# Ham3798/shielded-pool-pinocchio-solana

Hardware: AMD Instinct MI355X
Metric: Groth16 proofs/sec (higher is better)
Workload: dtype u32x8 (254-bit Montgomery integers); 1 GPU; audit_circuit (RLWE, const-PK; scripts/generate_audit.py:246-465), batch of 2048 independent proofs per GPU per step, every row a distinct witness; circuit=audit, n_constraints=29178, n_wires=35432, domain=32768, batch_per_gpu=2048, n_distinct_witnesses=2048, table_bytes=226725433344, parallelism=independent proofs x1, pk_bytes=9850060

## Files before the change

include/spp.h:

```cpp
#ifndef SPP_H
#define SPP_H
#include <stddef.h>
#include <stdint.h>
#ifdef __cplusplus
extern "C" {
#endif

#define SPP_OK 0
#define SPP_ERR_BAD_INPUT (-1)
#define SPP_ERR_NO_DEVICE (-2)
#define SPP_ERR_IO (-3)
#define SPP_ERR_UNSAT (-4)
#define SPP_ERR_HIP (-5)
#define SPP_ERR_NOT_IMPLEMENTED (-6)
#define SPP_ERR_FORMAT (-7)

#define SPP_CIRCUIT_WITHDRAW 1
#define SPP_CIRCUIT_AUDIT 2
#define SPP_CIRCUIT_WITHDRAW_REFSHAPE 3
#define SPP_CIRCUIT_WITHDRAW_DEPTH20 4

#define SPP_PROOF_LEN 388
#define SPP_WITHDRAW_PW_LEN 172
#define SPP_AUDIT_PW_LEN 76
// ... 172 lines not shown
int  spp_pool_withdraw_batch(spp_pool*, size_t count, const uint8_t* proofs, const uint8_t* pws, const uint8_t* recipients,
                             int32_t* result, uint64_t* amounts);
#define SPP_INSTR_DEPOSIT 0
#define SPP_INSTR_SUBMIT_AUDIT 1
#define SPP_INSTR_WITHDRAW 2
int  spp_pool_settle_log(spp_pool*, size_t count, const uint8_t* kinds,
                         size_t n_deposits, const uint8_t* roots,
                         size_t n_audits, const uint8_t* audit_proofs, const uint8_t* audit_pws,
                         size_t n_withdraws, const uint8_t* withdraw_proofs, const uint8_t* withdraw_pws, const uint8_t* recipients,
                         int32_t* result, uint64_t* amounts);

int spp_merkle_tree_find(spp_merkle_tree* t, size_t count, const uint8_t* leaves, const uint64_t* from, uint64_t* indices, uint32_t* matches);

#define SPP_WALLET_RECORD_LEN 160
#define SPP_WALLET_IN_TREE  1
#define SPP_WALLET_SPENT    2
#define SPP_WALLET_AUDITED  4
#define SPP_WALLET_REPEATED 8
int spp_wallet_sync(spp_merkle_tree* t, spp_pool* pool , size_t count, const uint8_t* deposits ,
                    const uint8_t* recipients , uint64_t* indices, uint32_t* flags,
                    uint8_t* records , uint8_t* notes );

int spp_ntt_fr(spp_ctx* ctx, uint8_t* data, uint32_t logn, int inverse);
int spp_msm_g1(spp_ctx* ctx, const uint8_t* bases, const uint8_t* scalars, size_t n, int window_bits, uint8_t out[64]);
int spp_msm_g2(spp_ctx* ctx, const uint8_t* bases, const uint8_t* scalars, size_t n, int window_bits, uint8_t out[128]);
int spp_msm_flat_unit(spp_ctx* ctx, int group, const uint8_t* bases, size_t n, const uint8_t* scalars, size_t P, int window_bits, uint8_t* out,
                      uint32_t* redo_lanes);

int spp_msm_g1_pippenger(spp_ctx* ctx, const uint8_t* bases, const uint8_t* scalars, size_t n, uint8_t out[64]);
int spp_msm_g2_pippenger(spp_ctx* ctx, const uint8_t* bases, const uint8_t* scalars, size_t n, uint8_t out[128]);
int spp_msm_g1_pippenger_bench(spp_ctx* ctx, size_t n, uint64_t seed, const uint8_t scale_be[32], int iters, uint8_t out[64],
                               float* ms_total, float* ms_bucket_kernel);
int spp_msm_g1_pippenger_bench_dist(spp_ctx* ctx, size_t n, uint64_t seed, uint32_t small_permille, const uint8_t scale_be[32], int iters,
                                    uint8_t out[64], float* ms_total, float* ms_bucket_kernel);
int spp_msm_g1_pippenger_bench_shard(spp_ctx* ctx, size_t n_total, size_t first, size_t count, uint64_t seed, uint32_t small_permille,
                                     const uint8_t scale_be[32], int iters, uint8_t out[64], float* ms_total, float* ms_bucket_kernel);

#ifdef __cplusplus
}
#endif
#endif
```

shielded-pool-pinocchio-solana_amd/csrc/kernels.hpp:

```cpp
#pragma once
#include <hip/hip_runtime.h>
#include <stdint.h>
#include "bn254.hpp"
#include "f29.hpp"
#include "msm_plan.hpp"
#include "msm_ragged.hpp"
#include "rlwe_ntt.hpp"

namespace spp {

struct DevSparse {
  const uint32_t* rowptr;
  const uint32_t* wire;
  const uint32_t* coeff;
  const uint32_t* lit;
};
static constexpr uint32_t COEFF_ONE = 0x80000000u;
static constexpr uint32_t COEFF_MINUS_ONE = 0x40000000u;
static constexpr uint32_t COEFF_MASK = 0x3fffffffu;

struct HashConsts {
  const Fr* pos3_rc;  const Fr* pos3_mds;
  const Fr* pos5_rc;  const Fr* pos5_mds;
  const Fr* p2_rc;    const Fr* p2_mu;
  const uint32_t* pos3_mds29;
  const uint32_t* pos5_mds29;
};
// ... 124 lines not shown
struct PoolSet;
struct PoolState;
void launch_pool_screen_audit(hipStream_t st, const PoolSet& audits, uint64_t salt, const uint8_t* pws, uint32_t count, int32_t* prov, uint32_t* list,
                              uint32_t* n_list);
void launch_pool_screen_withdraw(hipStream_t st, const PoolState* state, const PoolSet& audits, const PoolSet& nullifiers, uint64_t salt,
                                 const uint8_t* pws, const uint8_t* recipients, uint32_t count, int32_t* prov, uint64_t* amounts, uint32_t* list,
                                 uint32_t* n_list);
struct PoolLogView;
void launch_pool_screen_withdraw_log(hipStream_t st, const PoolLogView& view, const PoolSet& audits, const PoolSet& nullifiers, uint64_t salt,
                                     const uint8_t* pws, const uint8_t* recipients, const uint32_t* deposits_before, const uint32_t* audits_before,
                                     uint32_t count, int32_t* prov, uint64_t* amounts, uint32_t* list, uint32_t* n_list);
void launch_pool_scatter(hipStream_t st, const uint32_t* pos, uint32_t count, const int32_t* codes, int32_t* result, const uint64_t* amounts,
                         uint64_t* amounts_out);
void launch_pool_screen_import(hipStream_t st, const PoolSet& set, uint64_t salt, const uint8_t* keys, uint32_t count, int32_t* prov);
void launch_pool_contains(hipStream_t st, const PoolSet& set, uint64_t salt, const uint8_t* keys, uint32_t count, uint8_t* present);
void launch_pool_resolve(hipStream_t st, uint32_t* slots, uint32_t mask, uint64_t salt, const uint8_t* keys, uint32_t stride, uint32_t count,
                         const int32_t* prov, const int32_t* proof_ok, int32_t dup, int32_t* result);
void launch_pool_commit(hipStream_t st, const PoolSet& set, uint64_t salt, const uint8_t* keys, uint32_t stride, uint32_t count, const int32_t* result,
                        uint32_t* set_count);
void launch_spmv_check(hipStream_t st, DevCircuit dc, const Fr* W, Fr* abc, uint32_t n, uint32_t P, uint32_t* status, int16_t* small = nullptr);

void launch_ntt(hipStream_t st, Fr* data, uint32_t logn, uint32_t P, const Fr* tw, bool dif, uint32_t nbatch, size_t batch_stride,
                const Fr* post = nullptr);
void launch_scale_rows(hipStream_t st, Fr* data, const Fr* table, uint32_t n, uint32_t P, uint32_t nbatch, size_t batch_stride);
void launch_qap_pointwise(hipStream_t st, Fr* abc, uint32_t n, uint32_t P, Fr zinv);
void launch_qap_product(hipStream_t st, Fr* abc, uint32_t n, uint32_t P);

template <class F>
struct MsmWalk;
template <>
struct MsmWalk<Fq> {
  static constexpr uint32_t waves_per_simd = 3;
  static constexpr uint32_t rows_waves_per_simd = 2;
  static constexpr int product_form = F29_SCAN;
  static constexpr uint32_t occ(uint32_t Wt) { return Wt == 1 ? waves_per_simd : rows_waves_per_simd; }
};
template <>
struct MsmWalk<Fq2> {
  static constexpr uint32_t waves_per_simd = 2;
  static constexpr uint32_t rows_waves_per_simd = 1;
  static constexpr int product_form = F29_COLUMNS;
  static constexpr uint32_t occ(uint32_t Wt) { return Wt == 1 ? waves_per_simd : rows_waves_per_simd; }
};
template <class F>
void launch_build_table(hipStream_t st, const Affine<F>* bases, uint32_t N, uint32_t c, uint32_t Wt, uint32_t row0, uint32_t nrows,
                        Affine<F>* table, XYZZ<F>* tmp, F* tmp_pre, const MsmBlock* blocks = nullptr, uint32_t E = 0);
// ... 55 lines not shown
```

shielded-pool-pinocchio-solana_amd/csrc/kernels_ntt.hip:

```cpp
#include "kernels.hpp"

namespace spp {

static constexpr uint32_t NTT_TILE_ELEMS = 1024;
static constexpr uint32_t NTT_THREADS = 256;

template <bool DIF>
__global__ void __launch_bounds__(NTT_THREADS) k_ntt_pass(Fr* __restrict__ data, uint32_t logn, uint32_t P, const Fr* __restrict__ tw,
                                                          uint32_t s_lo, uint32_t s_hi, size_t batch_stride, const Fr* __restrict__ post) {
  extern __shared__ __align__(16) unsigned char smem_raw[];
  Fr* sh = reinterpret_cast<Fr*>(smem_raw);
  data += (size_t)blockIdx.y * batch_stride;
  const uint32_t n = 1u << logn;
  const uint32_t lg = s_hi - s_lo;
  const uint32_t G = 1u << lg;
  const uint32_t T = NTT_TILE_ELEMS / G;
  const uint32_t stride = DIF ? (n >> s_hi) : (1u << s_lo);
  const uint64_t Cq = (uint64_t)stride * P;
  const uint64_t ncols = ((uint64_t)n >> lg) * P;
  const uint64_t col0 = (uint64_t)blockIdx.x * T;
  const bool col_major = Cq >= T;

  if (col_major && T <= NTT_THREADS) {
    const uint32_t tc = threadIdx.x & (T - 1), jr = threadIdx.x / T, jstep = NTT_THREADS / T;
// ... 67 lines not shown
        sh[(j + half_l) * T + tc] = e ? d * tw[e] : d;
      } else {
        if (e) v = v * tw[e];
        sh[j * T + tc] = u + v;
        sh[(j + half_l) * T + tc] = u - v;
      }
    }
    __syncthreads();
  }

  for (uint32_t idx = threadIdx.x; idx < G * T; idx += NTT_THREADS) {
    uint32_t j, tc;
    if (col_major) { tc = idx % T; j = idx / T; } else { j = idx % G; tc = idx / G; }
    uint64_t col = col0 + tc;
    if (col < ncols) {
      uint64_t bh = col / Cq, q = col % Cq;
      Fr v = sh[j * T + tc];
      if (post) v = v * post[(uint32_t)(bh * G) * stride + j * stride + (uint32_t)(q / P)];
      data[bh * G * Cq + (uint64_t)j * Cq + q] = v;
    }
  }
}

void launch_ntt(hipStream_t st, Fr* data, uint32_t logn, uint32_t P, const Fr* tw, bool dif, uint32_t nbatch, size_t batch_stride,
                const Fr* post) {
  static bool attr_set = false;
  if (!attr_set) {
    (void)hipFuncSetAttribute((const void*)k_ntt_pass<true>, hipFuncAttributeMaxDynamicSharedMemorySize, (int)(NTT_TILE_ELEMS * sizeof(Fr)));
    (void)hipFuncSetAttribute((const void*)k_ntt_pass<false>, hipFuncAttributeMaxDynamicSharedMemorySize, (int)(NTT_TILE_ELEMS * sizeof(Fr)));
    attr_set = true;
  }
  uint32_t npass = (logn + 7) / 8;
  uint32_t s = 0;
  for (uint32_t ps = 0; ps < npass; ps++) {
    uint32_t lg = (logn - s + (npass - ps) - 1) / (npass - ps);
    uint32_t G = 1u << lg, T = NTT_TILE_ELEMS / G;
    uint64_t ncols = ((uint64_t)1 << (logn - lg)) * P;
    dim3 grid((uint32_t)((ncols + T - 1) / T), nbatch);
    size_t shmem = (size_t)NTT_TILE_ELEMS * sizeof(Fr);
    if (dif)
      hipLaunchKernelGGL(k_ntt_pass<true>, grid, dim3(NTT_THREADS), shmem, st, data, logn, P, tw, s, s + lg, batch_stride,
                         ps + 1 == npass ? post : (const Fr*)nullptr);
    else
      hipLaunchKernelGGL(k_ntt_pass<false>, grid, dim3(NTT_THREADS), shmem, st, data, logn, P, tw, s, s + lg, batch_stride,
                         ps + 1 == npass ? post : (const Fr*)nullptr);
    s += lg;
  }
}

__global__ void __launch_bounds__(256) k_scale_rows(Fr* __restrict__ data, const Fr* __restrict__ table, uint32_t n, uint32_t P,
                                                    size_t batch_stride) {
  data += (size_t)blockIdx.y * batch_stride;
  uint64_t total = (uint64_t)n * P;
  for (uint64_t g = (uint64_t)blockIdx.x * blockDim.x + threadIdx.x; g < total; g += (uint64_t)gridDim.x * blockDim.x) {
    uint32_t i = (uint32_t)(g / P);
    data[g] = data[g] * table[i];
  }
}
void launch_scale_rows(hipStream_t st, Fr* data, const Fr* table, uint32_t n, uint32_t P, uint32_t nbatch, size_t batch_stride) {
  uint64_t total = (uint64_t)n * P;
  uint32_t blocks = (uint32_t)((total + 255) / 256);
  if (blocks > 2048) blocks = 2048;
  hipLaunchKernelGGL(k_scale_rows, dim3(blocks, nbatch), dim3(256), 0, st, data, table, n, P, batch_stride);
}

__global__ void __launch_bounds__(256) k_qap_pointwise(Fr* __restrict__ abc, uint64_t total, Fr zinv) {
  Fr* a = abc;
  const Fr* b = abc + total;
// ... 24 lines not shown
```

shielded-pool-pinocchio-solana_amd/csrc/spp_circuit.hpp:

```cpp
#pragma once
#include "spp_internal.hpp"
#include "msm_classes.hpp"

template <class F>
struct MsmSet {
  uint32_t N = 0;
  Affine<F>* table = nullptr;
  uint32_t* rows = nullptr;
  bool from_h = false;
  uint32_t c = 0;
  uint32_t Wt = 0;
  MsmBlock* blocks = nullptr;
  bool narrow = false;
};
template <class F>
struct MsmBuf {
  XYZZ<F>* partial = nullptr;
  XYZZ<F>* out = nullptr;
  size_t partial_cap = 0;
  MsmPlan plan{};
};
struct Workspace {
  hipStream_t st = nullptr;
  hipStream_t st2 = nullptr;
// ... 50 lines not shown
  MsmTuning msm;
};
static constexpr uint64_t SCALED_BLIND_MAX_SCALARS = 1500000;
inline uint32_t scaled_blind_max_batch(uint32_t n_a, uint32_t n_b1) {
  const uint64_t n = (uint64_t)n_a + n_b1;
  return n ? (uint32_t)std::max<uint64_t>(1, std::min<uint64_t>(1024, SCALED_BLIND_MAX_SCALARS / n)) : 1;
}
struct spp_circuit {
  spp_ctx* ctx = nullptr;
  std::vector<SolveStep> schedule;
  Circuit circ;
  DevCircuit dc{};
  uint32_t c_bits = 10, n = 0, logn = 0;
  uint32_t max_batch_div = SOLVE_SCRATCH_MIN_ROWS;
  DevCoop coop{};
  Switches sw;
  bool generic_solver = false;
  uint32_t row_r = 0, row_s = 0, row_rs = 0, n_rows = 0;
  size_t in_stride = 0, pw_stride = 0;
  uint64_t table_bytes = 0;
  MsmSet<Fq> A, B1, K, Z, CB, CS;
  MsmSet<Fq2> B2;
  Fr *tw_fwd = nullptr, *tw_inv = nullptr, *coset_br = nullptr, *coset_inv_br = nullptr;
  Fr zinv;
  std::vector<void*> owned;
  Workspace ws[SPP_NWS];
  int next_ws = 0, last_ws = 0, prev_ws = 0;
  std::vector<PendingTable<Fq>> pending1;
  std::vector<PendingTable<Fq2>> pending2;
};

template <class T>
static int own_upload(spp_circuit* c, T** dst, const std::vector<T>& src) {
  HIP_TRY(dev_upload(dst, src));
  c->owned.push_back((void*)*dst);
  return 0;
}

#pragma GCC visibility push(hidden)
int coop_plan(spp_circuit* c);
int row_paths_plan(spp_circuit* c);
void destroy_circuit(spp_circuit* c);
void free_workspace(Workspace& w);
#pragma GCC visibility pop
```

shielded-pool-pinocchio-solana_amd/csrc/spp_load.cpp:

```cpp
#include "spp_circuit.hpp"

static std::vector<PendingTable<Fq>>& pending(spp_circuit* c, Fq*) { return c->pending1; }
static std::vector<PendingTable<Fq2>>& pending(spp_circuit* c, Fq2*) { return c->pending2; }

static int upload_sparse(spp_circuit* c, const Circuit& circ, const Sparse& m, DevSparse* out) {
  std::vector<uint32_t> wire(m.terms.size()), coeff(m.terms.size()), lit(m.terms.size(), 0);
  Fr one = Fr::one(), mone = Fr::one().neg();
  std::vector<uint32_t> small(circ.coeffs.size(), 0);
  for (size_t ci = 0; ci < circ.coeffs.size(); ci++) {
    uint32_t v[8], nv[8];
    circ.coeffs[ci].to_canonical(v);
    bool hi0 = true;
    for (int k = 1; k < 8; k++) hi0 = hi0 && v[k] == 0;
    if (hi0 && v[0] != 0 && v[0] < (1u << 28)) { small[ci] = v[0]; continue; }
    circ.coeffs[ci].neg().to_canonical(nv);
    hi0 = true;
    for (int k = 1; k < 8; k++) hi0 = hi0 && nv[k] == 0;
    if (hi0 && nv[0] != 0 && nv[0] < (1u << 28)) small[ci] = nv[0] | 0x80000000u;
  }
  for (size_t i = 0; i < m.terms.size(); i++) {
    wire[i] = m.terms[i].wire;
    uint32_t ci = m.terms[i].coeff;
    uint32_t flag = 0;
    if (circ.coeffs[ci] == one) flag = COEFF_ONE;
// ... 400 lines not shown
  for (uint32_t k = 0; k < n / 2; k++) {
    tf[k] = a;
    ti[k] = b;
    a = a * w;
    b = b * wi;
  }
  Fr g = c->sw.h_mode == 2 ? fr_root_of_unity(logn + 1) : Fr::from_u64(5), gi = g.inv(), ninv = Fr::from_u64(n).inv();
  std::vector<Fr> gp(n), gip(n);
  Fr x = ninv, y = ninv;
  for (uint32_t i = 0; i < n; i++) {
    gp[i] = x;
    gip[i] = y;
    x = x * g;
    y = y * gi;
  }
  for (uint32_t pos = 0; pos < n; pos++) {
    uint32_t i = bitrev(pos, logn);
    cb[pos] = gp[i];
    cib[pos] = gip[i];
  }
  if ((e = own_upload(c, &c->tw_fwd, tf)) || (e = own_upload(c, &c->tw_inv, ti)) || (e = own_upload(c, &c->coset_br, cb)) ||
      (e = own_upload(c, &c->coset_inv_br, cib)))
    return e;
  Fr gn = g.pow_u64(n);
  c->zinv = (gn - Fr::one()).inv();
  return 0;
}

static int load_key_sets(spp_circuit* c, const LoadState& s) {
  const PkFile& pk = s.pk;
  const uint32_t* cw = s.cw;
  const bool* flat = s.flat;
  int e;
  {
    std::vector<uint32_t> w = pk.A_w;
    std::vector<G1Affine> p = pk.A;
    merge_point(w, p, 0u, pk.alpha1);
    w.push_back(c->row_r); p.push_back(pk.delta1);
    if ((e = make_set(c, &c->A, w, p, false, cw[0], flat[0], msm_base_bounds(s.wc, w)))) return e;
  }
  {
    std::vector<uint32_t> w = pk.B1_w;
    std::vector<G1Affine> p = pk.B1;
    merge_point(w, p, 0u, pk.beta1);
    w.push_back(c->row_s); p.push_back(pk.delta1);
    if ((e = make_set(c, &c->B1, w, p, false, cw[1], flat[1], msm_base_bounds(s.wc, w)))) return e;
// ... 426 lines not shown
```

shielded-pool-pinocchio-solana_amd/csrc/spp_micro_api.cpp:

```cpp
#include "spp_internal.hpp"
#include "arith_probe.hpp"

extern "C" int spp_ntt_fr(spp_ctx* ctx, uint8_t* data, uint32_t logn, int inverse) {
  if (!ctx || !data || logn == 0 || logn > 24) return fail(SPP_ERR_BAD_INPUT, "bad argument");
  std::lock_guard<std::mutex> lk(ctx->mu);
  HIP_TRY(hipSetDevice(ctx->device));
  const uint32_t n = 1u << logn;
  Fr w = fr_root_of_unity(logn);
  if (inverse) w = w.inv();
  std::vector<Fr> tw(n / 2 ? n / 2 : 1), host(n);
  Fr a = Fr::one();
  for (uint32_t k = 0; k < n / 2; k++) { tw[k] = a; a = a * w; }
  for (uint32_t i = 0; i < n; i++) host[i] = Fr::from_bytes_be(data + 32 * (size_t)i);
  DevBuf d_tw, d_x;
  HIP_TRY(d_tw.alloc(sizeof(Fr) * tw.size()));
  HIP_TRY(d_x.alloc(sizeof(Fr) * n));
  HIP_TRY(hipMemcpy(d_tw.p, tw.data(), sizeof(Fr) * tw.size(), hipMemcpyHostToDevice));
  HIP_TRY(hipMemcpy(d_x.p, host.data(), sizeof(Fr) * n, hipMemcpyHostToDevice));
  launch_ntt(ctx->stream, d_x.as<Fr>(), logn, 1, d_tw.as<Fr>(), true, 1, 0);
  HIP_TRY(hipStreamSynchronize(ctx->stream));
  HIP_TRY(hipGetLastError());
  HIP_TRY(hipMemcpy(host.data(), d_x.p, sizeof(Fr) * n, hipMemcpyDeviceToHost));
  Fr ninv = inverse ? Fr::from_u64(n).inv() : Fr::one();
  for (uint32_t pos = 0; pos < n; pos++) {
    Fr v = host[pos];
    if (inverse) v = v * ninv;
    v.to_bytes_be(data + 32 * (size_t)bitrev(pos, logn));
  }
  return SPP_OK;
}

extern "C" int spp_debug_arith(spp_ctx* ctx, uint32_t selector, uint32_t arg, size_t n, const uint32_t* in, size_t in_words, uint32_t* out,
                               size_t out_words) {
  if (!ctx || !in || !out) return fail(SPP_ERR_BAD_INPUT, "NULL argument");
  if (n == 0 || n > ((size_t)1 << 20)) return fail(SPP_ERR_BAD_INPUT, "n must be in [1, 2^20]");
  uint32_t iw = 0, ow = 0;
  if (!arith_probe_shape(selector, &iw, &ow)) return fail(SPP_ERR_BAD_INPUT, "unknown selector 0x%x", selector);
  if (!arith_probe_arg_ok(selector, arg)) return fail(SPP_ERR_BAD_INPUT, "selector 0x%x does not know arg %u", selector, arg);
  if (in_words != iw || out_words != ow)
    return fail(SPP_ERR_BAD_INPUT, "selector 0x%x takes %u words and returns %u per case", selector, iw, ow);
  std::lock_guard<std::mutex> lk(ctx->mu);
  HIP_TRY(hipSetDevice(ctx->device));
  hipStream_t st = ctx->stream;
  DevBuf d_in, d_out;
  UP(d_in, in, n * iw * sizeof(uint32_t));
  HIP_TRY(d_out.alloc(n * ow * sizeof(uint32_t)));
  if (!launch_arith_probe(st, selector, arg, d_in.as<uint32_t>(), d_out.as<uint32_t>(), (uint32_t)n))
    return fail(SPP_ERR_BAD_INPUT, "unknown selector 0x%x", selector);
  HIP_TRY(hipGetLastError());
  HIP_TRY(hipStreamSynchronize(st));
  HIP_TRY(hipMemcpy(out, d_out.p, n * ow * sizeof(uint32_t), hipMemcpyDeviceToHost));
// ... 141 lines not shown
```

shielded-pool-pinocchio-solana_amd/csrc/spp_prove.cpp:

```cpp
#include "spp_circuit.hpp"

template <class T>
static int ws_alloc(Workspace& w, T** p, size_t count) {
  HIP_TRY(hipMalloc((void**)p, sizeof(T) * std::max<size_t>(count, 1)));
  w.owned.push_back((void*)*p);
  return 0;
}
template <class F>
static int ws_set(const spp_circuit* c, Workspace& w, const MsmSet<F>* s, MsmBuf<F>* b, size_t P) {
  b->partial_cap = msm_partial_cap(s->N, P, s->c, s->Wt, MsmWalk<F>::occ(s->Wt), c->sw.msm);
  int e;
  if ((e = ws_alloc(w, &b->partial, b->partial_cap))) return e;
  return ws_alloc(w, &b->out, P);
}
static int ensure_workspace(spp_circuit* c, Workspace& w, size_t P) {
  if (P <= w.cap) return 0;
  HIP_TRY(hipStreamSynchronize(w.st));
  free_workspace(w);
  int e;
  if ((e = ws_alloc(w, &w.W, (size_t)c->n_rows * P)) || (e = ws_alloc(w, &w.abc, (size_t)3 * c->n * P)) ||
      (e = ws_alloc(w, &w.scratch, (size_t)c->max_batch_div * P)) || (e = ws_alloc(w, &w.commit_affine, P)) ||
      (e = ws_alloc(w, &w.d_inputs, c->in_stride * P)) || (e = ws_alloc(w, &w.d_rs, 64 * P)) ||
      (e = ws_alloc(w, &w.d_proofs, (size_t)SPP_PROOF_LEN * P)) || (e = ws_alloc(w, &w.d_pws, c->pw_stride * P)) ||
      (e = ws_alloc(w, &w.d_status, P)) || (e = ws_alloc(w, &w.counters, 256 * P)))
// ... 74 lines not shown
          } else launch_solve_coop(st, c->dc, c->coop, w.W, w.scratch, tr, P);
        }
        else launch_solve(st, c->dc, w.W, w.scratch, s.a, s.b, P);
        break;
      case SolveStep::BATCH_DIV: launch_batch_div(st, c->dc, w.W, w.scratch, s.a, s.b, P); break;
      case SolveStep::COUNT8: launch_count8(st, c->dc, w.W, w.counters, s.a, s.b, s.c, P); break;
      case SolveStep::COMMIT:
        run_msm(c, w, c->CB, w.CB, P, true);
        launch_challenge(st, w.CB.out, w.W, circ.challenge_wire, P, w.commit_affine, d_status);
        break;
    }
  }
  hipEventRecord(w.ev[1], st);
  hipEventRecord(w.ev_w, st);
  hipStream_t side = (w.st2 != w.st && w.own_st2p && P > c->sw.coop_max_batch) ? w.own_st2p : w.st2;
  if (c->sw.no_side && P <= c->sw.coop_max_batch) side = st;
  hipStreamWaitEvent(side, w.ev_w, 0);
  run_msm(c, w, c->B2, w.B2, P, false, side, &w.g2_ev);
  hipEventRecord(w.ev_b2, side);
  launch_spmv_check(st, c->dc, w.W, w.abc, n, P, d_status, w.small);
  hipEventRecord(w.ev[2], st);
  const size_t bs = (size_t)n * P;
  const uint32_t nt = c->sw.h_mode == 2 ? 2 : 3;
  launch_ntt(st, w.abc, c->logn, P, c->tw_inv, true, nt, bs, c->coset_br);
  launch_ntt(st, w.abc, c->logn, P, c->tw_fwd, false, nt, bs);
  if (c->sw.h_mode == 2) launch_qap_product(st, w.abc, n, P);
  else launch_qap_pointwise(st, w.abc, n, P, c->zinv);
  if (c->sw.h_mode == 0) launch_ntt(st, w.abc, c->logn, P, c->tw_inv, true, 1, bs, c->coset_inv_br);
  hipEventRecord(w.ev[3], st);
  {
    MsmFoldSets<Fq> fs{};
    const MsmSet<Fq>* sets[7] = {&c->A, &c->B1, &c->K, &c->Z, &c->CS, &c->A, &c->B1};
    MsmBuf<Fq>* bufs[7] = {&w.A, &w.B1, &w.K, &w.Z, &w.CS, &w.sA, &w.rB};
    const Fr* scal[7] = {nullptr, nullptr, nullptr, nullptr, nullptr, w.Ws, w.Wr};
    const int nsets = scaled_blind ? 7 : 5;
    if (scaled_blind) launch_scale_witness(st, w.W, w.Ws, w.Wr, c->n_rows, c->row_r, c->row_s, P);
    for (int i = 0; i < nsets; i++) {
      run_msm(c, w, *sets[i], *bufs[i], P, i < 5, nullptr, nullptr, false, scal[i]);
      fs.partial[i] = bufs[i]->partial;
      fs.out[i] = bufs[i]->out;
      fs.Sg[i] = sets[i]->N ? bufs[i]->plan.Sg : 0;
      fs.R[i] = bufs[i]->plan.R;
      fs.c[i] = sets[i]->c;
    }
    launch_msm_reduce_multi<Fq>(st, fs, nsets, P);
  }
  hipEventRecord(w.ev[4], st);
  hipStreamWaitEvent(st, w.ev_b2, 0);
  hipEventRecord(w.ev[5], st);
  AssembleArgs a;
  a.mA = w.A.out; a.mB1 = w.B1.out; a.mB2 = w.B2.out; a.mK = w.K.out; a.mZ = w.Z.out; a.mPok = w.CS.out;
// ... 416 lines not shown
```

shielded-pool-pinocchio-solana_amd/spp/lib.py:

```python
import ctypes
import os

_HERE = os.path.dirname(os.path.abspath(__file__))
LIB_PATH = os.path.join(os.path.dirname(_HERE), "libspp.so")
_LIB = None

SPP_OK = 0
SPP_ERR_BAD_INPUT = -1
SPP_ERR_UNSAT = -4
SPP_CIRCUIT_WITHDRAW = 1
SPP_CIRCUIT_AUDIT = 2
SPP_CIRCUIT_WITHDRAW_DEPTH20 = 4
SPP_CIRCUIT_WITHDRAW_REFSHAPE = 3
PROOF_LEN = 388
NOTE_LEN = 160
DEPOSIT_LEN = 96
AUDIT_PW_LEN = 76
SPP_RLC_SERIAL_TAIL = 1
SPP_RLC_NO_FALLBACK = 2
SPP_AUDIT_BAD_PROOF = 1
SPP_AUDIT_BAD_CIPHERTEXT = 2
SPP_AUDIT_BAD_IDENTITY = 4
WITHDRAW_PW_LEN = 172
SPP_POOL_STATE_LEN = 1072
# ... 110 lines not shown
    L.spp_pool_set_verifier.argtypes = [vp, i32, u32]
    L.spp_pool_verify_stats.argtypes = [vp, ctypes.POINTER(u32)]
    L.spp_pool_new.argtypes = [vp, cp, sz, cp, sz, ctypes.c_uint64, ctypes.POINTER(vp)]
    L.spp_pool_free.argtypes = [vp]
    L.spp_pool_free.restype = None
    L.spp_pool_add_roots.argtypes = [vp, sz, cp]
    L.spp_pool_state.argtypes = [vp, vp]
    L.spp_pool_counts.argtypes = [vp, vp]
    L.spp_pool_import_keys.argtypes = [vp, i32, sz, cp]
    L.spp_pool_contains.argtypes = [vp, i32, sz, cp, vp]
    L.spp_pool_submit_audit_batch.argtypes = [vp, sz, cp, cp, vp]
    L.spp_pool_withdraw_batch.argtypes = [vp, sz, cp, cp, cp, vp, vp]
    L.spp_pool_settle_log.argtypes = [vp, sz, cp, sz, cp, sz, cp, cp, sz, cp, cp, cp, vp, vp]
    L.spp_withdraw_rows_from_tree.argtypes = [vp, sz, cp, vp]
    L.spp_prove_withdraw_notes_device.argtypes = [vp, vp, sz, vp, vp, vp, vp, vp]
    L.spp_prove_withdraw_notes.argtypes = [vp, vp, sz, cp, cp, vp, vp, vp]
    L.spp_shamir_reconstruct.argtypes = [vp, u32, vp, cp, sz, vp, vp]
    L.spp_rlwe_decrypt_batch.argtypes = [vp, vp, sz, vp, vp, vp]
    L.spp_rlwe_sample_key.argtypes = [sz, u32, vp, vp, vp]
    L.spp_rlwe_keygen_batch.argtypes = [vp, sz, vp, vp, vp, vp, vp]
    L.spp_rlwe_key_check.argtypes = [vp, sz, vp, vp, vp, vp]
    L.spp_shamir_split.argtypes = [vp, u32, u32, vp, sz, cp, cp, vp]
    L.spp_ntt_fr.argtypes = [vp, vp, u32, i32]
    L.spp_msm_g1.argtypes = [vp, cp, cp, sz, i32, vp]
    L.spp_msm_g2.argtypes = [vp, cp, cp, sz, i32, vp]
    L.spp_msm_flat_unit.argtypes = [vp, i32, cp, sz, cp, sz, i32, vp, ctypes.POINTER(ctypes.c_uint32)]
    L.spp_msm_g1_pippenger.argtypes = [vp, cp, cp, sz, vp]
    L.spp_msm_g2_pippenger.argtypes = [vp, cp, cp, sz, vp]
    L.spp_msm_g1_pippenger_bench.argtypes = [vp, sz, ctypes.c_uint64, cp, i32, vp, ctypes.POINTER(ctypes.c_float), ctypes.POINTER(ctypes.c_float)]
    L.spp_msm_g1_pippenger_bench_dist.argtypes = [vp, sz, ctypes.c_uint64, ctypes.c_uint32, cp, i32, vp, ctypes.POINTER(ctypes.c_float),
                                                  ctypes.POINTER(ctypes.c_float)]
    L.spp_msm_g1_pippenger_bench_shard.argtypes = [vp, sz, sz, sz, ctypes.c_uint64, ctypes.c_uint32, cp, i32, vp, ctypes.POINTER(ctypes.c_float),
                                                   ctypes.POINTER(ctypes.c_float)]
    _LIB = L
    return L


def last_error():
    return load_library().spp_last_error().decode()


def check(rc):
    if rc != 0:
        raise SppError(rc, last_error())
```

shielded-pool-pinocchio-solana_amd/spp/prover.py:

```python
import ctypes
import numpy as np
from .lib import load_library, check, SppError, PROOF_LEN, SPP_ERR_UNSAT, AUDIT_PW_LEN


def build_circuit(circuit_id, out_path, aux=None):
    L = load_library()
    n = ctypes.c_uint32(0)
    auxbuf = None
    if aux is not None:
        auxbuf = (ctypes.c_uint32 * len(aux))(*[int(v) for v in aux])
    check(L.spp_circuit_build(int(circuit_id), auxbuf, out_path.encode(), ctypes.byref(n)))
    return n.value


def verify(vk_bytes, proof_bytes, pw_bytes):
    L = load_library()
    ok = ctypes.c_int(0)
    check(L.spp_verify(vk_bytes, len(vk_bytes), proof_bytes, len(proof_bytes), pw_bytes, len(pw_bytes), ctypes.byref(ok)))
    return bool(ok.value)


def pairing_check_host(pairs):
    L = load_library()
    ok = ctypes.c_int(0)
# ... 19 lines not shown

    def load_circuit(self, circuit_path, pk_path, window_bits=0, bits=None):
        return CircuitHandle(self, circuit_path, pk_path, window_bits, bits)

    def plan_windows(self, pk_paths, budget_bytes=240e9):
        n = len(pk_paths)
        sizes = (ctypes.c_uint32 * (7 * n))()
        for k, path in enumerate(pk_paths):
            one = (ctypes.c_uint32 * 7)()
            check(self.L.spp_pk_msm_sizes(path.encode(), one))
            sizes[7 * k:7 * k + 7] = list(one)
        bits = (ctypes.c_uint32 * (7 * n))()
        check(self.L.spp_plan_windows(n, sizes, float(budget_bytes), bits))
        return [list(bits[7 * k:7 * k + 7]) for k in range(n)]

    def ntt(self, values, inverse=False):
        n = len(values)
        logn = n.bit_length() - 1
        assert 1 << logn == n
        buf = ctypes.create_string_buffer(b"".join(int(v).to_bytes(32, "big") for v in values), 32 * n)
        check(self.L.spp_ntt_fr(self.h, ctypes.cast(buf, ctypes.c_void_p), logn, 1 if inverse else 0))
        raw = buf.raw
        return [int.from_bytes(raw[32 * i:32 * i + 32], "big") for i in range(n)]

    def debug_arith(self, selector, rows, out_words, arg=0):
        a = np.ascontiguousarray(rows, dtype=np.uint32)
        assert a.ndim == 2
        out = np.empty((a.shape[0], int(out_words)), dtype=np.uint32)
        check(self.L.spp_debug_arith(self.h, int(selector), int(arg), a.shape[0], a.ctypes.data_as(ctypes.c_void_p), a.shape[1],
                                     out.ctypes.data_as(ctypes.c_void_p), out.shape[1]))
        return out

    def msm_g1(self, bases_bytes, scalars, window_bits=8):
        n = len(scalars)
        out = ctypes.create_string_buffer(64)
        sc = b"".join(int(s).to_bytes(32, "big") for s in scalars)
        check(self.L.spp_msm_g1(self.h, bases_bytes, sc, n, int(window_bits), ctypes.cast(out, ctypes.c_void_p)))
        return out.raw

    def msm_g2(self, bases_bytes, scalars, window_bits=8):
        out = ctypes.create_string_buffer(128)
        sc = b"".join(int(s).to_bytes(32, "big") for s in scalars)
        check(self.L.spp_msm_g2(self.h, bases_bytes, sc, len(scalars), int(window_bits), ctypes.cast(out, ctypes.c_void_p)))
        return out.raw

    def msm_flat(self, group, bases_bytes, scalar_rows, window_bits=8):
# ... 252 lines not shown
```

Before: 7369 proofs/s.

## Run QAP NTT passes in 29-bit limb arithmetic with lazy reduction

Adds an NTT pass kernel that converts Fr values to a nine-limb 29-bit representation in LDS, runs butterflies with lazy additions, and fully reduces only on selected sweep stages. Twiddle and coset tables are precomputed in the 29-bit form at load time. The prover's H-polynomial NTTs now use this path, falling back to the old kernel when a pass's tile shape does not fit. The aim is to cut the cost of Montgomery multiplies and reductions per butterfly, in exchange for larger LDS tiles (36 bytes per element), lower occupancy, and extra conversion at load and store.

Result: no change. 7401 proofs/s (median of 6 runs) (+0.4%).

```diff
diff --git a/include/spp.h b/include/spp.h
--- a/include/spp.h
+++ b/include/spp.h
@@ -218,6 +218,7 @@
                     uint8_t* records , uint8_t* notes );
 
 int spp_ntt_fr(spp_ctx* ctx, uint8_t* data, uint32_t logn, int inverse);
+int spp_ntt_fr_batch(spp_ctx* ctx, uint8_t* data, uint32_t logn, uint32_t P, uint32_t nbatch, int inverse, int with_post);
 int spp_msm_g1(spp_ctx* ctx, const uint8_t* bases, const uint8_t* scalars, size_t n, int window_bits, uint8_t out[64]);
 int spp_msm_g2(spp_ctx* ctx, const uint8_t* bases, const uint8_t* scalars, size_t n, int window_bits, uint8_t out[128]);
 int spp_msm_flat_unit(spp_ctx* ctx, int group, const uint8_t* bases, size_t n, const uint8_t* scalars, size_t P, int window_bits, uint8_t* out,
diff --git a/profiles/ntt29_accounting.py b/profiles/ntt29_accounting.py
--- /dev/null
+++ b/profiles/ntt29_accounting.py
@@ -0,0 +1,91 @@
+#!/usr/bin/env python3
+import re
+import sys
+
+LDS = {"k_ntt_pass": 1024 * 32, "k_ntt29_pass": 1024 * 36}
+
+
+def kernels(text):
+    out = {}
+    lines = text.split("\n")
+    i = 0
+    while i < len(lines):
+        m = re.match(r"^(_ZN3spp\w+):\s*(;.*)?$", lines[i])
+        if m:
+            j = i + 1
+            while j < len(lines) and "s_endpgm" not in lines[j]:
+                j += 1
+            while j + 1 < len(lines) and not lines[j + 1].startswith(".Lfunc_end"):
+                j += 1
+            res = {}
+            for k in range(j, min(len(lines), j + 120)):
+                for key, pat in (("vgpr", r"; NumVgprs: (\d+)"), ("scratch", r"; ScratchSize: (\d+)"), ("occ", r"; Occupancy: (\d+)")):
+                    mm = re.match(pat, lines[k])
+                    if mm and key not in res:
+                        res[key] = int(mm.group(1))
+            out[m.group(1)] = (lines[i + 1:j], res)
+            i = j
+        i += 1
+    return out
+
+
+def butterfly_loops(body):
+    blocks = [("", [], [])]
+    for line in body:
+        s = line.strip()
+        m = re.match(r"^(\.LBB\w+):", s)
+        if m:
+            blocks.append((m.group(1), [], []))
+        elif s and not s.startswith((".", ";")) and not s.split()[0].endswith(":"):
+            blocks[-1][1].append(s.split()[0])
+            if s.startswith(("s_cbranch", "s_branch")):
+                blocks[-1][2].append(s.split()[1])
+    index = {b[0]: n for n, b in enumerate(blocks)}
+    loops = [(index[t], n) for n, (_, _, targets) in enumerate(blocks) for t in targets if t in index and index[t] <= n]
+    found = []
+    for n, (_, ops, _) in enumerate(blocks):
+        if ops.count("v_mad_u64_u32") < 100:
+            continue
+        around = [lp for lp in loops if lp[0] <= n <= lp[1]]
+        if not around:
+            continue
+        lo, hi = min(around, key=lambda lp: lp[1] - lp[0])
+        if (lo, hi) not in [f[0] for f in found]:
+            found.append(((lo, hi), [op for b in blocks[lo:hi + 1] for op in b[1]]))
+    return [ops for _, ops in found]
+
+
+def pretty(sym):
+    for name in ("k_ntt29_pass", "k_ntt_pass"):
+        tag = "%d%sILb" % (len(name), name)
+        if tag in sym:
+            dif = sym.split(tag)[1][0] == "1"
+            return name, "%s<%s>" % (name, "DIF" if dif else "DIT")
+    return None, None
+
+
+def main():
+    print("%-8s %-20s %-18s %6s %4s %7s %6s %6s %5s %6s %5s %8s %5s %6s" % ("listing", "kernel", "loop", "instr", "per", "instr/1", "mad64", "mul32", "lds", "gload", "VGPR", "scratch", "waves", "LDS B"))
+    for arg in sys.argv[1:]:
+        label, path = arg.split(":", 1)
+        for sym, (body, res) in sorted(kernels(open(path).read()).items()):
+            base, name = pretty(sym)
+            if not name:
+                continue
+            for ops in butterfly_loops(body):
+                mad = ops.count("v_mad_u64_u32")
+                per = max(1, round(mad / 170.0))
+                if any(op.startswith("global_store") for op in ops):
+                    kind = "post"
+                elif base == "k_ntt_pass":
+                    kind = "butterfly"
+                else:
+                    kind = "plain+sweep" if per >= 4 else "plain" if mad / per <= 170 else "sweep"
+                path = "generic" if any("rcp" in op for op in ops) else "tile"
+                print("%-8s %-20s %-18s %6d %4d %7.1f %6d %6d %5d %6d %5s %8s %5s %6d" % (
+                    label, name, kind + "/" + path, len(ops), per, len(ops) / per, mad, ops.count("v_mul_lo_u32"),
+                    sum(1 for op in ops if op.startswith("ds_")), sum(1 for op in ops if op.startswith("global_load")),
+                    res.get("vgpr"), res.get("scratch"), res.get("occ"), LDS[base]))
+
+if __name__ == "__main__":
+    main()
diff --git a/profiles/ntt29_batches.py b/profiles/ntt29_batches.py
--- /dev/null
+++ b/profiles/ntt29_batches.py
@@ -0,0 +1,28 @@
+#!/usr/bin/env python3
+import csv
+import glob
+import json
+import os
+import sys
+
+
+def main():
+    d, out = sys.argv[1], sys.argv[2]
+    path = glob.glob(os.path.join(d, "**", "*kernel_trace.csv"), recursive=True)[0]
+    rows = []
+    with open(path) as f:
+        for r in csv.DictReader(f):
+            if "k_ntt" in r["Kernel_Name"] and "pass" in r["Kernel_Name"]:
+                rows.append((int(r["Start_Timestamp"]), int(r["End_Timestamp"]) - int(r["Start_Timestamp"]), r["Kernel_Name"]))
+    rows.sort()
+    per = 4
+    sums = [round(sum(x[1] for x in rows[i:i + per]) / 1e6, 4) for i in range(0, len(rows) - per + 1, per)]
+    names = sorted(set(x[2].split("(")[0] for x in rows))
+    res = {"kernels": names, "launches": len(rows), "launches_per_batch": per, "batches": len(sums), "ms_per_batch": sums,
+           "mean_ms": round(sum(sums) / len(sums), 4), "min_ms": min(sums), "max_ms": max(sums), "range_ms": round(max(sums) - min(sums), 4)}
+    json.dump(res, open(out, "w"), indent=1)
+    print(json.dumps(res))
+
+
+if __name__ == "__main__":
+    main()
diff --git a/shielded-pool-pinocchio-solana_amd/csrc/kernels.hpp b/shielded-pool-pinocchio-solana_amd/csrc/kernels.hpp
--- a/shielded-pool-pinocchio-solana_amd/csrc/kernels.hpp
+++ b/shielded-pool-pinocchio-solana_amd/csrc/kernels.hpp
@@ -3,6 +3,7 @@
 #include <stdint.h>
 #include "bn254.hpp"
 #include "f29.hpp"
+#include "ntt29.hpp"
 #include "msm_plan.hpp"
 #include "msm_ragged.hpp"
 #include "rlwe_ntt.hpp"
@@ -173,6 +174,8 @@
 
 void launch_ntt(hipStream_t st, Fr* data, uint32_t logn, uint32_t P, const Fr* tw, bool dif, uint32_t nbatch, size_t batch_stride,
                 const Fr* post = nullptr);
+void launch_ntt29(hipStream_t st, Fr* data, uint32_t logn, uint32_t P, const Fr* tw, const F29<FrParams>* tw29, bool dif, uint32_t nbatch,
+                  size_t batch_stride, const Fr* post = nullptr, const F29<FrParams>* post29 = nullptr);
 void launch_scale_rows(hipStream_t st, Fr* data, const Fr* table, uint32_t n, uint32_t P, uint32_t nbatch, size_t batch_stride);
 void launch_qap_pointwise(hipStream_t st, Fr* abc, uint32_t n, uint32_t P, Fr zinv);
 void launch_qap_product(hipStream_t st, Fr* abc, uint32_t n, uint32_t P);
diff --git a/shielded-pool-pinocchio-solana_amd/csrc/kernels_ntt.hip b/shielded-pool-pinocchio-solana_amd/csrc/kernels_ntt.hip
--- a/shielded-pool-pinocchio-solana_amd/csrc/kernels_ntt.hip
+++ b/shielded-pool-pinocchio-solana_amd/csrc/kernels_ntt.hip
@@ -1,4 +1,5 @@
 #include "kernels.hpp"
+#include "ntt29.hpp"
 
 namespace spp {
 
@@ -113,28 +114,158 @@
   }
 }
 
-void launch_ntt(hipStream_t st, Fr* data, uint32_t logn, uint32_t P, const Fr* tw, bool dif, uint32_t nbatch, size_t batch_stride,
-                const Fr* post) {
+static void launch_ntt_pass(hipStream_t st, Fr* data, uint32_t logn, uint32_t P, const Fr* tw, bool dif, uint32_t nbatch, size_t batch_stride,
+                            uint32_t s, uint32_t lg, const Fr* post) {
   static bool attr_set = false;
   if (!attr_set) {
     (void)hipFuncSetAttribute((const void*)k_ntt_pass<true>, hipFuncAttributeMaxDynamicSharedMemorySize, (int)(NTT_TILE_ELEMS * sizeof(Fr)));
     (void)hipFuncSetAttribute((const void*)k_ntt_pass<false>, hipFuncAttributeMaxDynamicSharedMemorySize, (int)(NTT_TILE_ELEMS * sizeof(Fr)));
     attr_set = true;
   }
+  const uint32_t G = 1u << lg, T = NTT_TILE_ELEMS / G;
+  const uint64_t ncols = ((uint64_t)1 << (logn - lg)) * P;
+  dim3 grid((uint32_t)((ncols + T - 1) / T), nbatch);
+  const size_t shmem = (size_t)NTT_TILE_ELEMS * sizeof(Fr);
+  if (dif) hipLaunchKernelGGL(k_ntt_pass<true>, grid, dim3(NTT_THREADS), shmem, st, data, logn, P, tw, s, s + lg, batch_stride, post);
+  else hipLaunchKernelGGL(k_ntt_pass<false>, grid, dim3(NTT_THREADS), shmem, st, data, logn, P, tw, s, s + lg, batch_stride, post);
+}
+
+void launch_ntt(hipStream_t st, Fr* data, uint32_t logn, uint32_t P, const Fr* tw, bool dif, uint32_t nbatch, size_t batch_stride,
+                const Fr* post) {
   uint32_t npass = (logn + 7) / 8;
   uint32_t s = 0;
   for (uint32_t ps = 0; ps < npass; ps++) {
     uint32_t lg = (logn - s + (npass - ps) - 1) / (npass - ps);
-    uint32_t G = 1u << lg, T = NTT_TILE_ELEMS / G;
-    uint64_t ncols = ((uint64_t)1 << (logn - lg)) * P;
-    dim3 grid((uint32_t)((ncols + T - 1) / T), nbatch);
-    size_t shmem = (size_t)NTT_TILE_ELEMS * sizeof(Fr);
-    if (dif)
-      hipLaunchKernelGGL(k_ntt_pass<true>, grid, dim3(NTT_THREADS), shmem, st, data, logn, P, tw, s, s + lg, batch_stride,
-                         ps + 1 == npass ? post : (const Fr*)nullptr);
-    else
-      hipLaunchKernelGGL(k_ntt_pass<false>, grid, dim3(NTT_THREADS), shmem, st, data, logn, P, tw, s, s + lg, batch_stride,
-                         ps + 1 == npass ? post : (const Fr*)nullptr);
+    launch_ntt_pass(st, data, logn, P, tw, dif, nbatch, batch_stride, s, lg, ps + 1 == npass ? post : (const Fr*)nullptr);
+    s += lg;
+  }
+}
+
+static constexpr uint32_t NTT29_LDS_BYTES = NTT_TILE_ELEMS * 36;
+
+struct Ntt29Tile {
+  uint4* a;
+  uint4* b;
+  uint32_t* c;
+  __device__ __forceinline__ explicit Ntt29Tile(unsigned char* raw)
+      : a(reinterpret_cast<uint4*>(raw)), b(reinterpret_cast<uint4*>(raw) + NTT_TILE_ELEMS),
+        c(reinterpret_cast<uint32_t*>(raw + 32 * NTT_TILE_ELEMS)) {}
+  __device__ __forceinline__ Ntt29::F get(uint32_t i) const {
+    const uint4 x = a[i], y = b[i];
+    Ntt29::F r;
+    r.l[0] = x.x; r.l[1] = x.y; r.l[2] = x.z; r.l[3] = x.w;
+    r.l[4] = y.x; r.l[5] = y.y; r.l[6] = y.z; r.l[7] = y.w;
+    r.l[8] = c[i];
+    return r;
+  }
+  __device__ __forceinline__ void put(uint32_t i, const Ntt29::F& v) const {
+    a[i] = make_uint4(v.l[0], v.l[1], v.l[2], v.l[3]);
+    b[i] = make_uint4(v.l[4], v.l[5], v.l[6], v.l[7]);
+    c[i] = v.l[8];
+  }
+};
+
+template <bool DIF, bool SWEEP>
+__device__ __forceinline__ void ntt29_stage(const Ntt29Tile& sh, const Ntt29::F* __restrict__ tw, uint32_t t, uint32_t lg, uint32_t logn,
+                                            uint32_t stride, uint32_t base_low, uint32_t T, uint32_t tc, uint32_t jr, uint32_t jstep) {
+  const uint32_t half_l = Ntt29::half_len<DIF>(t, lg);
+  const uint32_t mult_log = Ntt29::mult_log(logn, half_l, stride);
+  static_assert(NTT_TILE_ELEMS == 4 * NTT_THREADS, "two butterflies per lane and stage");
+  if constexpr (DIF) {
+    for (uint32_t jj = jr; jj < 2 * jstep; jj += jstep) {
+      uint32_t lo;
+      const uint32_t j = Ntt29::upper(jj, half_l, lo);
+      const Ntt29::F w = tw[(lo * stride + base_low) << mult_log];
+      Ntt29::F u = sh.get(j * T + tc);
+      Ntt29::F v = sh.get((j + half_l) * T + tc);
+      Ntt29::dif<SWEEP>(u, v, w);
+      sh.put(j * T + tc, u);
+      sh.put((j + half_l) * T + tc, v);
+    }
+  } else {
+    uint32_t iu[2], iv[2];
+    Ntt29::F u[2], v[2], w[2];
+    SPP_UNROLL for (int b = 0; b < 2; b++) {
+      uint32_t lo;
+      const uint32_t j = Ntt29::upper(jr + b * jstep, half_l, lo);
+      w[b] = tw[(lo * stride + base_low) << mult_log];
+      iu[b] = j * T + tc;
+      iv[b] = (j + half_l) * T + tc;
+      u[b] = sh.get(iu[b]);
+      v[b] = sh.get(iv[b]);
+    }
+    SPP_UNROLL for (int b = 0; b < 2; b++) Ntt29::dit<SWEEP>(u[b], v[b], w[b]);
+    SPP_UNROLL for (int b = 0; b < 2; b++) {
+      sh.put(iu[b], u[b]);
+      sh.put(iv[b], v[b]);
+    }
+  }
+}
+
+template <bool DIF>
+__global__ void __launch_bounds__(NTT_THREADS) __attribute__((amdgpu_waves_per_eu(4))) k_ntt29_pass(Fr* __restrict__ data, uint32_t logn, uint32_t P, const Ntt29::F* __restrict__ tw,
+                                                            uint32_t s_lo, uint32_t s_hi, size_t batch_stride,
+                                                            const Ntt29::F* __restrict__ post) {
+  extern __shared__ __align__(16) unsigned char smem_raw[];
+  const Ntt29Tile sh(smem_raw);
+  data += (size_t)blockIdx.y * batch_stride;
+  const uint32_t n = 1u << logn;
+  const uint32_t lg = s_hi - s_lo;
+  const uint32_t G = 1u << lg;
+  const uint32_t T = NTT_TILE_ELEMS / G;
+  const uint32_t stride = DIF ? (n >> s_hi) : (1u << s_lo);
+  const uint64_t Cq = (uint64_t)stride * P;
+  const uint64_t ncols = ((uint64_t)n >> lg) * P;
+  const uint32_t tc = threadIdx.x & (T - 1), jr = threadIdx.x / T, jstep = NTT_THREADS / T;
+  const uint64_t col = (uint64_t)blockIdx.x * T + tc;
+  const bool valid = col < ncols;
+  const uint64_t bh = valid ? col / Cq : 0, q = valid ? col % Cq : 0;
+  const uint32_t base_low = (uint32_t)(q / P);
+  Fr* ptr = data + bh * G * Cq + q;
+  if (valid)
+    for (uint32_t j = jr; j < G; j += jstep) sh.put(j * T + tc, Ntt29::load(ptr[(uint64_t)j * Cq]));
+  __syncthreads();
+  for (uint32_t t = 0; t < lg; t++) {
+    if (valid) {
+      if (Ntt29::sweeps<DIF>(t, lg)) ntt29_stage<DIF, true>(sh, tw, t, lg, logn, stride, base_low, T, tc, jr, jstep);
+      else ntt29_stage<DIF, false>(sh, tw, t, lg, logn, stride, base_low, T, tc, jr, jstep);
+    }
+    __syncthreads();
+  }
+  if (valid) {
+    if (post) {
+      const uint32_t row0 = (uint32_t)(bh * G) * stride + base_low;
+      for (uint32_t j = jr; j < G; j += jstep) ptr[(uint64_t)j * Cq] = Ntt29::store_post(sh.get(j * T + tc), post[row0 + j * stride]);
+    } else {
+      for (uint32_t j = jr; j < G; j += jstep) ptr[(uint64_t)j * Cq] = Ntt29::store(sh.get(j * T + tc));
+    }
+  }
+}
+
+void launch_ntt29(hipStream_t st, Fr* data, uint32_t logn, uint32_t P, const Fr* tw, const Ntt29::F* tw29, bool dif, uint32_t nbatch,
+                  size_t batch_stride, const Fr* post, const Ntt29::F* post29) {
+  static bool attr_set = false;
+  if (!attr_set) {
+    (void)hipFuncSetAttribute((const void*)k_ntt29_pass<true>, hipFuncAttributeMaxDynamicSharedMemorySize, (int)NTT29_LDS_BYTES);
+    (void)hipFuncSetAttribute((const void*)k_ntt29_pass<false>, hipFuncAttributeMaxDynamicSharedMemorySize, (int)NTT29_LDS_BYTES);
+    attr_set = true;
+  }
+  const uint32_t npass = (logn + 7) / 8;
+  uint32_t s = 0;
+  for (uint32_t ps = 0; ps < npass; ps++) {
+    const uint32_t lg = (logn - s + (npass - ps) - 1) / (npass - ps);
+    const uint32_t G = 1u << lg, T = NTT_TILE_ELEMS / G;
+    const uint64_t stride = dif ? ((uint64_t)1 << (logn - s - lg)) : ((uint64_t)1 << s);
+    const bool last = ps + 1 == npass;
+    if (stride * P >= T && T <= NTT_THREADS) {
+      const uint64_t ncols = ((uint64_t)1 << (logn - lg)) * P;
+      dim3 grid((uint32_t)((ncols + T - 1) / T), nbatch);
+      const Ntt29::F* p29 = last && post ? post29 : nullptr;
+      if (dif) hipLaunchKernelGGL(k_ntt29_pass<true>, grid, dim3(NTT_THREADS), NTT29_LDS_BYTES, st, data, logn, P, tw29, s, s + lg, batch_stride, p29);
+      else hipLaunchKernelGGL(k_ntt29_pass<false>, grid, dim3(NTT_THREADS), NTT29_LDS_BYTES, st, data, logn, P, tw29, s, s + lg, batch_stride, p29);
+    } else {
+      launch_ntt_pass(st, data, logn, P, tw, dif, nbatch, batch_stride, s, lg, last ? post : (const Fr*)nullptr);
+    }
     s += lg;
   }
 }
diff --git a/shielded-pool-pinocchio-solana_amd/csrc/ntt29.hpp b/shielded-pool-pinocchio-solana_amd/csrc/ntt29.hpp
--- /dev/null
+++ b/shielded-pool-pinocchio-solana_amd/csrc/ntt29.hpp
@@ -0,0 +1,88 @@
+#pragma once
+#include "f29.hpp"
+
+namespace spp {
+
+struct Ntt29 {
+  using F = F29<FrParams>;
+  using Pm = FrParams;
+  static constexpr int FORM = F29_COLUMNS;
+  static constexpr uint32_t M = F::M;
+
+  static SPP_HD constexpr uint32_t KP9(uint32_t mult, int k) {
+    uint64_t carry = 0, limb = 0;
+    for (int i = 0; i <= k; i++) {
+      const uint64_t t = (uint64_t)mult * F::P9(i) + carry;
+      limb = i < 8 ? (t & M) : t;
+      carry = t >> 29;
+    }
+    return (uint32_t)limb;
+  }
+  static SPP_HD constexpr uint32_t SUBC_8P_2(int k) { return k < 8 ? KP9(8, k) + (2u << 29) - (k ? 2u : 0u) : KP9(8, 8) - 2u; }
+  static SPP_HD constexpr uint32_t NEGP9(int k) { return (M - F::P9(k)) + (k == 0 ? 1u : 0u); }
+  static constexpr uint64_t RECIP = (1ull << 53) / ((uint64_t)F::P9(8) + 1u);
+
+  static SPP_HD F reduce(const F& x) {
+    uint32_t q = (uint32_t)(((uint64_t)x.l[8] * RECIP) >> 53);
+    F::Base::hide24(q);
+    F r;
+    uint64_t carry = 0;
+    SPP_UNROLL for (int k = 0; k < 9; k++) {
+      const uint64_t t = (uint64_t)q * NEGP9(k) + carry + x.l[k];
+      r.l[k] = (uint32_t)t & M;
+      carry = t >> 29;
+    }
+    return r;
+  }
+
+  static SPP_HD F load(const Fr& a) { return F::from_words(a.l); }
+  static SPP_HD Fr store(const F& x) {
+    Fr r;
+    x.to_words(r.l);
+    return r;
+  }
+  static SPP_HD Fr store_post(const F& x, const F& post) {
+    Fr r;
+    F::template mul_as<FORM>(x, post).to_words(r.l);
+    return r;
+  }
+  template <bool SWEEP>
+  static SPP_HD void dif(F& u, F& v, const F& tw) {
+    const F s = add_lazy(u, v);
+    if constexpr (SWEEP) {
+      const F dl = F::template sub_lazy<SUBC_8P_2>(u, v);
+      u = reduce(s);
+      v = F::template mul_as<FORM>(dl, tw);
+    } else {
+      const F dl = F::template sub_lazy<Pm::SUBC_4P_1>(u, v);
+      u = s;
+      v = F::template mul_as<FORM>(dl, tw);
+    }
+  }
+  template <bool SWEEP>
+  static SPP_HD void dit(F& u, F& v, const F& tw) {
+    const F t = F::template mul_as<FORM>(v, tw);
+    const F s = add_lazy(u, t);
+    const F dl = F::template sub_lazy<Pm::SUBC_2P_1>(u, t);
+    u = SWEEP ? reduce(s) : s;
+    v = SWEEP ? reduce(dl) : dl;
+  }
+  template <bool DIF>
+  static SPP_HD bool sweeps(uint32_t t, uint32_t lg) { return t + 1 == lg || (DIF ? (t & 1u) == 1u : t % 3u == 2u); }
+  static SPP_HD F to_tw(const Fr& a) {
+    const Fr c = (a * Fr::from_u64(32)).canonical();
+    return F::from_words(c.l);
+  }
+
+  template <bool DIF>
+  static SPP_HD uint32_t half_len(uint32_t t, uint32_t lg) { return DIF ? ((1u << lg) >> (t + 1)) : (1u << t); }
+  static SPP_HD uint32_t mult_log(uint32_t logn, uint32_t half_l, uint32_t stride) {
+    return logn - 1 - (31 - (uint32_t)__builtin_clz(half_l)) - (31 - (uint32_t)__builtin_clz(stride));
+  }
+  static SPP_HD uint32_t upper(uint32_t jj, uint32_t half_l, uint32_t& lo) {
+    lo = jj & (half_l - 1);
+    return ((jj - lo) << 1) + lo;
+  }
+};
+
+}
diff --git a/shielded-pool-pinocchio-solana_amd/csrc/spp_circuit.hpp b/shielded-pool-pinocchio-solana_amd/csrc/spp_circuit.hpp
--- a/shielded-pool-pinocchio-solana_amd/csrc/spp_circuit.hpp
+++ b/shielded-pool-pinocchio-solana_amd/csrc/spp_circuit.hpp
@@ -96,6 +96,7 @@
   MsmSet<Fq> A, B1, K, Z, CB, CS;
   MsmSet<Fq2> B2;
   Fr *tw_fwd = nullptr, *tw_inv = nullptr, *coset_br = nullptr, *coset_inv_br = nullptr;
+  F29<FrParams> *tw_fwd29 = nullptr, *tw_inv29 = nullptr, *coset_br29 = nullptr, *coset_inv_br29 = nullptr;
   Fr zinv;
   std::vector<void*> owned;
   Workspace ws[SPP_NWS];
diff --git a/shielded-pool-pinocchio-solana_amd/csrc/spp_load.cpp b/shielded-pool-pinocchio-solana_amd/csrc/spp_load.cpp
--- a/shielded-pool-pinocchio-solana_amd/csrc/spp_load.cpp
+++ b/shielded-pool-pinocchio-solana_amd/csrc/spp_load.cpp
@@ -446,6 +446,13 @@
   if ((e = own_upload(c, &c->tw_fwd, tf)) || (e = own_upload(c, &c->tw_inv, ti)) || (e = own_upload(c, &c->coset_br, cb)) ||
       (e = own_upload(c, &c->coset_inv_br, cib)))
     return e;
+  const std::vector<Fr>* src[4] = {&tf, &ti, &cb, &cib};
+  F29<FrParams>** dst[4] = {&c->tw_fwd29, &c->tw_inv29, &c->coset_br29, &c->coset_inv_br29};
+  for (int k = 0; k < 4; k++) {
+    std::vector<F29<FrParams>> t29(src[k]->size());
+    for (size_t i = 0; i < t29.size(); i++) t29[i] = Ntt29::to_tw((*src[k])[i]);
+    if ((e = own_upload(c, dst[k], t29))) return e;
+  }
   Fr gn = g.pow_u64(n);
   c->zinv = (gn - Fr::one()).inv();
   return 0;
diff --git a/shielded-pool-pinocchio-solana_amd/csrc/spp_micro_api.cpp b/shielded-pool-pinocchio-solana_amd/csrc/spp_micro_api.cpp
--- a/shielded-pool-pinocchio-solana_amd/csrc/spp_micro_api.cpp
+++ b/shielded-pool-pinocchio-solana_amd/csrc/spp_micro_api.cpp
@@ -27,6 +27,51 @@
     if (inverse) v = v * ninv;
     v.to_bytes_be(data + 32 * (size_t)bitrev(pos, logn));
   }
+  return SPP_OK;
+}
+
+extern "C" int spp_ntt_fr_batch(spp_ctx* ctx, uint8_t* data, uint32_t logn, uint32_t P, uint32_t nbatch, int inverse, int with_post) {
+  if (!ctx || !data || logn == 0 || logn > 24 || P == 0 || nbatch == 0) return fail(SPP_ERR_BAD_INPUT, "bad argument");
+  const uint64_t n = (uint64_t)1 << logn, total = n * P * nbatch;
+  if (P > ((uint64_t)1 << 24) || nbatch > ((uint64_t)1 << 24) || n * P > ((uint64_t)1 << 24) || total > ((uint64_t)1 << 24))
+    return fail(SPP_ERR_BAD_INPUT, "n * P * nbatch must be at most 2^24");
+  std::lock_guard<std::mutex> lk(ctx->mu);
+  HIP_TRY(hipSetDevice(ctx->device));
+  Fr w = fr_root_of_unity(logn);
+  if (inverse) w = w.inv();
+  std::vector<Fr> tw(n / 2), post(n), host(total);
+  std::vector<Ntt29::F> tw29(n / 2), post29(n);
+  Fr a = Fr::one();
+  for (uint64_t k = 0; k < n / 2; k++) { tw[k] = a; tw29[k] = Ntt29::to_tw(a); a = a * w; }
+  a = inverse ? Fr::from_u64(n).inv() : Fr::one();
+  for (uint32_t i = 0; i < n; i++) {
+    const uint32_t pos = inverse ? bitrev(i, logn) : i;
+    post[pos] = a;
+    post29[pos] = Ntt29::to_tw(a);
+    a = a * Fr::from_u64(5);
+  }
+  for (uint32_t b = 0; b < nbatch; b++)
+    for (uint32_t i = 0; i < n; i++) {
+      const uint32_t pos = inverse ? i : bitrev(i, logn);
+      for (uint32_t p = 0; p < P; p++) host[((size_t)b * n + pos) * P + p] = Fr::from_bytes_be(data + 32 * (((size_t)b * n + i) * P + p));
+    }
+  hipStream_t st = ctx->stream;
+  DevBuf d_tw, d_tw29, d_post, d_post29, d_x;
+  UP(d_tw, tw.data(), sizeof(Fr) * tw.size());
+  UP(d_tw29, tw29.data(), sizeof(Ntt29::F) * tw29.size());
+  UP(d_post, post.data(), sizeof(Fr) * post.size());
+  UP(d_post29, post29.data(), sizeof(Ntt29::F) * post29.size());
+  UP(d_x, host.data(), sizeof(Fr) * host.size());
+  launch_ntt29(st, d_x.as<Fr>(), logn, P, d_tw.as<Fr>(), d_tw29.as<Ntt29::F>(), inverse != 0, nbatch, (size_t)n * P,
+               with_post ? d_post.as<Fr>() : nullptr, with_post ? d_post29.as<Ntt29::F>() : nullptr);
+  HIP_TRY(hipGetLastError());
+  HIP_TRY(hipStreamSynchronize(ctx->stream));
+  HIP_TRY(hipMemcpy(host.data(), d_x.p, sizeof(Fr) * host.size(), hipMemcpyDeviceToHost));
+  for (uint32_t b = 0; b < nbatch; b++)
+    for (uint32_t i = 0; i < n; i++) {
+      const uint32_t pos = inverse ? bitrev(i, logn) : i;
+      for (uint32_t p = 0; p < P; p++) host[((size_t)b * n + pos) * P + p].to_bytes_be(data + 32 * (((size_t)b * n + i) * P + p));
+    }
   return SPP_OK;
 }
 
diff --git a/shielded-pool-pinocchio-solana_amd/csrc/spp_prove.cpp b/shielded-pool-pinocchio-solana_amd/csrc/spp_prove.cpp
--- a/shielded-pool-pinocchio-solana_amd/csrc/spp_prove.cpp
+++ b/shielded-pool-pinocchio-solana_amd/csrc/spp_prove.cpp
@@ -120,11 +120,12 @@
   hipEventRecord(w.ev[2], st);
   const size_t bs = (size_t)n * P;
   const uint32_t nt = c->sw.h_mode == 2 ? 2 : 3;
-  launch_ntt(st, w.abc, c->logn, P, c->tw_inv, true, nt, bs, c->coset_br);
-  launch_ntt(st, w.abc, c->logn, P, c->tw_fwd, false, nt, bs);
+  launch_ntt29(st, w.abc, c->logn, P, c->tw_inv, c->tw_inv29, true, nt, bs, c->coset_br, c->coset_br29);
+  launch_ntt29(st, w.abc, c->logn, P, c->tw_fwd, c->tw_fwd29, false, nt, bs);
   if (c->sw.h_mode == 2) launch_qap_product(st, w.abc, n, P);
   else launch_qap_pointwise(st, w.abc, n, P, c->zinv);
-  if (c->sw.h_mode == 0) launch_ntt(st, w.abc, c->logn, P, c->tw_inv, true, 1, bs, c->coset_inv_br);
+  if (c->sw.h_mode == 0)
+    launch_ntt29(st, w.abc, c->logn, P, c->tw_inv, c->tw_inv29, true, 1, bs, c->coset_inv_br, c->coset_inv_br29);
   hipEventRecord(w.ev[3], st);
   {
     MsmFoldSets<Fq> fs{};
diff --git a/shielded-pool-pinocchio-solana_amd/spp/lib.py b/shielded-pool-pinocchio-solana_amd/spp/lib.py
--- a/shielded-pool-pinocchio-solana_amd/spp/lib.py
+++ b/shielded-pool-pinocchio-solana_amd/spp/lib.py
@@ -156,6 +156,7 @@
     L.spp_rlwe_key_check.argtypes = [vp, sz, vp, vp, vp, vp]
     L.spp_shamir_split.argtypes = [vp, u32, u32, vp, sz, cp, cp, vp]
     L.spp_ntt_fr.argtypes = [vp, vp, u32, i32]
+    L.spp_ntt_fr_batch.argtypes = [vp, vp, u32, u32, u32, i32, i32]
     L.spp_msm_g1.argtypes = [vp, cp, cp, sz, i32, vp]
     L.spp_msm_g2.argtypes = [vp, cp, cp, sz, i32, vp]
     L.spp_msm_flat_unit.argtypes = [vp, i32, cp, sz, cp, sz, i32, vp, ctypes.POINTER(ctypes.c_uint32)]
diff --git a/shielded-pool-pinocchio-solana_amd/spp/prover.py b/shielded-pool-pinocchio-solana_amd/spp/prover.py
--- a/shielded-pool-pinocchio-solana_amd/spp/prover.py
+++ b/shielded-pool-pinocchio-solana_amd/spp/prover.py
@@ -65,6 +65,12 @@
         check(self.L.spp_ntt_fr(self.h, ctypes.cast(buf, ctypes.c_void_p), logn, 1 if inverse else 0))
         raw = buf.raw
         return [int.from_bytes(raw[32 * i:32 * i + 32], "big") for i in range(n)]
+
+    def ntt_batch(self, data, logn, P, nbatch, inverse=False, with_post=False):
+        assert len(data) == 32 * nbatch * (1 << logn) * P
+        buf = ctypes.create_string_buffer(bytes(data), len(data))
+        check(self.L.spp_ntt_fr_batch(self.h, ctypes.cast(buf, ctypes.c_void_p), logn, P, nbatch, 1 if inverse else 0, 1 if with_post else 0))
+        return buf.raw
 
     def debug_arith(self, selector, rows, out_words, arg=0):
         a = np.ascontiguousarray(rows, dtype=np.uint32)
```
